# CyberAgentAILab/layout-dm

Hardware: NVIDIA H100
Metric: layouts_per_sec_T100_batch1024_N25 (higher is better)
Workload: dtype fp16

## Files before the change

layoutdm_b200/csrc/common.cuh:

```cuda
#pragma once
#include <cuda.h>
#include <cuda_bf16.h>
#include <cuda_fp16.h>
#include <cuda_runtime.h>
#include <stdint.h>

namespace ldm {

#define LDM_DEVINL __device__ __forceinline__

constexpr float kLogEps = -69.07755278982137f;

LDM_DEVINL uint32_t smem_u32(const void* p) { return static_cast<uint32_t>(__cvta_generic_to_shared(p)); }
LDM_DEVINL void st_shared_u32(uint32_t addr, uint32_t v) { asm volatile("st.shared.u32 [%0], %1;" ::"r"(addr), "r"(v) : "memory"); }

LDM_DEVINL void pdl_wait() { asm volatile("griddepcontrol.wait;" ::: "memory"); }
LDM_DEVINL void pdl_launch_dependents() { asm volatile("griddepcontrol.launch_dependents;" ::: "memory"); }
LDM_DEVINL void pdl_sync() { pdl_wait(); pdl_launch_dependents(); }

LDM_DEVINL void mbar_init(uint64_t* bar, uint32_t count) {
  asm volatile("mbarrier.init.shared::cta.b64 [%0], %1;" ::"r"(smem_u32(bar)), "r"(count) : "memory");
}
LDM_DEVINL void fence_mbar_init() { asm volatile("fence.mbarrier_init.release.cluster;" ::: "memory"); }

// ... 3 lines not shown
LDM_DEVINL void mbar_arrive(uint64_t* bar) {
  asm volatile("mbarrier.arrive.shared::cta.b64 _, [%0];" ::"r"(smem_u32(bar)) : "memory");
}
LDM_DEVINL bool mbar_try_wait(uint64_t* bar, uint32_t parity) {
  uint32_t ok;
  asm volatile(
      "{\n\t.reg .pred p;\n\t"
      "mbarrier.try_wait.parity.shared::cta.b64 p, [%1], %2;\n\t"
      "selp.u32 %0, 1, 0, p;\n\t}\n"
      : "=r"(ok)
      : "r"(smem_u32(bar)), "r"(parity)
      : "memory");
  return ok != 0;
}
LDM_DEVINL void mbar_wait(uint64_t* bar, uint32_t parity) {
  uint32_t spins = 0;
  while (!mbar_try_wait(bar, parity)) {
    if (++spins > (1u << 28)) { asm volatile("trap;"); }
  }
}

LDM_DEVINL void tma_prefetch_desc(const CUtensorMap* m) {
  asm volatile("prefetch.tensormap [%0];" ::"l"(reinterpret_cast<uint64_t>(m)) : "memory");
}
LDM_DEVINL void tma_load_2d(void* smem_dst, const CUtensorMap* map, uint64_t* bar, int32_t c0, int32_t c1) {
  asm volatile(
      "cp.async.bulk.tensor.2d.shared::cluster.global.mbarrier::complete_tx::bytes [%0], [%1, {%3, %4}], [%2];"
      ::"r"(smem_u32(smem_dst)), "l"(reinterpret_cast<uint64_t>(map)), "r"(smem_u32(bar)), "r"(c0), "r"(c1)
      : "memory");
}
LDM_DEVINL void tma_store_2d(const CUtensorMap* map, const void* smem_src, int32_t c0, int32_t c1) {
  asm volatile("cp.async.bulk.tensor.2d.global.shared::cta.bulk_group [%0, {%2, %3}], [%1];"
               ::"l"(reinterpret_cast<uint64_t>(map)), "r"(smem_u32(smem_src)), "r"(c0), "r"(c1)
               : "memory");
}
LDM_DEVINL void bulk_copy_g2s(void* smem_dst, const void* src, uint32_t bytes, uint64_t* bar) {
  asm volatile("cp.async.bulk.shared::cluster.global.mbarrier::complete_tx::bytes [%0], [%1], %2, [%3];"
               ::"r"(smem_u32(smem_dst)), "l"(reinterpret_cast<uint64_t>(src)), "r"(bytes), "r"(smem_u32(bar))
               : "memory");
}
LDM_DEVINL void bulk_copy_s2g(void* dst, const void* smem_src, uint32_t bytes) {
  asm volatile("cp.async.bulk.global.shared::cta.bulk_group [%0], [%1], %2;"
               ::"l"(reinterpret_cast<uint64_t>(dst)), "r"(smem_u32(smem_src)), "r"(bytes)
               : "memory");
}
LDM_DEVINL void bulk_commit_group() { asm volatile("cp.async.bulk.commit_group;" ::: "memory"); }
template <int N>
LDM_DEVINL void bulk_wait_group_read() { asm volatile("cp.async.bulk.wait_group.read %0;" ::"n"(N) : "memory"); }
LDM_DEVINL void bulk_wait_group_all() { asm volatile("cp.async.bulk.wait_group 0;" ::: "memory"); }
LDM_DEVINL void fence_proxy_async_smem() { asm volatile("fence.proxy.async.shared::cta;" ::: "memory"); }

template <int R>
LDM_DEVINL void setmaxnreg_inc() { asm volatile("setmaxnreg.inc.sync.aligned.u32 %0;" ::"n"(R)); }
template <int R>
LDM_DEVINL void setmaxnreg_dec() { asm volatile("setmaxnreg.dec.sync.aligned.u32 %0;" ::"n"(R)); }

LDM_DEVINL uint32_t cluster_ctarank() { uint32_t r; asm volatile("mov.u32 %0, %%cluster_ctarank;" : "=r"(r)); return r; }
LDM_DEVINL uint32_t cluster_id_x() { uint32_t r; asm volatile("mov.u32 %0, %%clusterid.x;" : "=r"(r)); return r; }
LDM_DEVINL uint32_t cluster_count_x() { uint32_t r; asm volatile("mov.u32 %0, %%nclusterid.x;" : "=r"(r)); return r; }
LDM_DEVINL void cluster_sync() {
  asm volatile("barrier.cluster.arrive.release;\n\tbarrier.cluster.wait.acquire;" ::: "memory");
}
LDM_DEVINL uint32_t map_peer(const void* p, uint32_t rank) {
  uint32_t r;
  asm volatile("mapa.shared::cluster.u32 %0, %1, %2;" : "=r"(r) : "r"(smem_u32(p)), "r"(rank));
  return r;
}
LDM_DEVINL void st_async_f32(uint32_t addr, float v, uint32_t bar) {
  asm volatile("st.async.shared::cluster.mbarrier::complete_tx::bytes.f32 [%0], %1, [%2];" ::"r"(addr), "f"(v), "r"(bar) : "memory");
}

LDM_DEVINL void named_bar_sync(int id, int nthreads) { asm volatile("bar.sync %0, %1;" ::"r"(id), "r"(nthreads) : "memory"); }
LDM_DEVINL void named_bar_arrive(int id, int nthreads) { asm volatile("bar.arrive %0, %1;" ::"r"(id), "r"(nthreads) : "memory"); }

LDM_DEVINL void wgmma_fence() { asm volatile("wgmma.fence.sync.aligned;" ::: "memory"); }
LDM_DEVINL void wgmma_commit() { asm volatile("wgmma.commit_group.sync.aligned;" ::: "memory"); }
// ... 232 lines not shown
```

layoutdm_b200/csrc/gemm_tc.cuh:

```cuda
#pragma once
#include "common.cuh"

namespace ldm {

constexpr int kBM = 128;
constexpr int kWgK = 16;
constexpr int kGemmConsumers = 256;
constexpr int kProducerRegs = 40, kConsumerRegs = 232;

constexpr int gemm_kb(bool split) { return split ? 32 : 64; }

enum : int { EPI_QKV = 0, EPI_RELU = 1, EPI_F32 = 2, EPI_LN = 3 };

struct GemmParams {
  int M, N, K;
  int n_tiles;
  const float* bias;
  void* out;
  int ldo;
  float qscale;
  int qcols;
  const float* resid;
  float* y_out;
  const float* ln_scale;
// ... 427 lines not shown
#pragma unroll
      for (int cb = 0; cb < kCols / 64; ++cb) {
        if (n0 + cb * 64 >= p.N) continue;
        if (leader) bulk_wait_group_read<0>();
        wg_bar();
#pragma unroll
        for (int j8 = 8 * cb; j8 < 8 * cb + 8; ++j8) {
          const int c = col0 + 8 * j8;
          const uint32_t blk = stage_u32 + ((((j8 & 7) << 4) ^ sw) | (4 * (lane & 3)));
#pragma unroll
          for (int h = 0; h < 2; ++h) {
            float v[4];
            bias_act<EPI>(acc[h], j8, p.bias, c, scale, v);
            st_shared_u32(blk + (h * 64 + rw) * 128, O::pack(v[0], v[1]));
            st_shared_u32(blk + (h * 64 + rw + 8) * 128, O::pack(v[2], v[3]));
          }
        }
        fence_proxy_async_smem();
        wg_bar();
        if (leader) {
          tma_store_2d(&map_out, stage, n0 + cb * 64, m0);
          bulk_commit_group();
        }
      }
    }
    if (!mine_any) {
      for (int kb = 0; kb < num_kb; ++kb) { mbar_wait(&a_full[kb], ip); mbar_arrive(&a_empty[kb]); }
    }
  }
  if (leader) bulk_wait_group_all();
}

constexpr int kLnThreads = 384, kLnEpiThreads = 96;
template <int STAGES>
struct LnSmem {
  static constexpr int kRows = kBM, kCols = 232, kPairCols = 2 * kCols;
  using R = Ring<32, 1, kRows, kCols, 1, STAGES, false>;
  static constexpr int kLd = kCols;
  static constexpr int kOffBuf = R::kBytes;
  static constexpr int kOffBars = kOffBuf + kRows * kLd * 4;
  static constexpr int kOffStat = kOffBars + 128;
  static constexpr int kBytes = kOffStat + 9 * kRows * 4 + 1024 ;
  static_assert(2 * R::kStages * 8 + 6 * 8 <= 128, "barrier block overflow");
  static_assert(kLd * 4 % 16 == 0 && kLd * 4 % 128 == 32, "bulk copies need 16-byte aligned rows; fragment accesses need rows 32 mod 128 bytes");
  static_assert(kRows * kCols * 4 < (1 << 20), "a tile's residual bytes exceed the mbarrier transaction count");
};

template <int MODE, int STAGES>
__global__ void __launch_bounds__(kLnThreads, 1)
gemm_ln_kernel(const __grid_constant__ OpMaps<MODE> map_a , const __grid_constant__ OpMaps<MODE> map_b ,
               const GemmParams p) {
  static_assert(!kOpSplit<MODE>, "the split mode runs the fragment-epilogue LN GEMM");
  using SM = LnSmem<STAGES>;
  using O = OpT<MODE>;
  constexpr int kRows = SM::kRows, kCols = SM::kCols, kLd = SM::kLd, kAcc = kCols / 2;
  constexpr int kEpi = kGemmConsumers, kProducer = kEpi + kLnEpiThreads;

  extern __shared__ __align__(1024) uint8_t smem_raw[];
  uint8_t* smem = reinterpret_cast<uint8_t*>((reinterpret_cast<uintptr_t>(smem_raw) + 1023) & ~uintptr_t(1023));
  typename SM::R ring(smem, reinterpret_cast<uint64_t*>(smem + SM::kOffBars));
  uint64_t* res_full = ring.empty + SM::R::kStages;
  uint64_t* buf_full = res_full + 1;
  uint64_t* xs_full = buf_full + 1;
  uint64_t* xv_full = xs_full + 2;
  float* buf = reinterpret_cast<float*>(smem + SM::kOffBuf);
  float* s_piv = reinterpret_cast<float*>(smem + SM::kOffStat);
  float* s_own = s_piv + kRows;
  float* s_sum = s_own + kRows;
  float* v_own = s_sum + kRows;
  float* s_rstd = v_own + kRows;
  float* x_sum = s_rstd + kRows;
  float* x_var = x_sum + 2 * kRows;

  const int warp = __shfl_sync(0xffffffffu, threadIdx.x >> 5, 0), lane = threadIdx.x & 31;
  const int N = p.N;
  const int num_kb = SM::R::num_kb(p.K);
  const int n_work = p.M / kRows;
  const uint32_t rank = cluster_ctarank();
  const int col0 = kCols * static_cast<int>(rank);
  const int cl = static_cast<int>(cluster_id_x()), n_cl = static_cast<int>(cluster_count_x());
  const auto tile_m0 = [&](int t) { return (p.rev ? n_work - 1 - t : t) * kRows; };
  const uint32_t peer = rank ^ 1;
  const uint32_t px_sum = map_peer(x_sum, peer), pxs_full = map_peer(xs_full, peer);

  if (threadIdx.x == kProducer) {
    ring.prefetch(map_a, map_b);
    ring.init();
    mbar_init(res_full, 1);
    mbar_init(buf_full, kGemmConsumers);
    for (int b = 0; b < 2; ++b) { mbar_init(&xs_full[b], 1); mbar_init(&xv_full[b], 1); }
    fence_mbar_init();
  }
  cluster_sync();
  pdl_sync();

  if (threadIdx.x >= kProducer) {
    if (threadIdx.x == kProducer) {
      uint32_t phase = 0;
      int s = 0;
      for (int t = cl; t < n_work; t += n_cl) ring.load_tile(s, phase, map_a, map_b, num_kb, tile_m0(t), col0);
    }
  } else if (threadIdx.x >= kEpi) {
    const int et = threadIdx.x - kEpi;
    const bool copier = et < 32;
    constexpr uint32_t kRowBytes = kCols * sizeof(float);
    const float inv_n = 1.0f / static_cast<float>(N);
    constexpr int kVec = kCols / 4;
    constexpr int kTotal = kRows * kVec;
    constexpr int kPerThread = (kTotal + kLnEpiThreads - 1) / kLnEpiThreads;
    const uint32_t px_var = map_peer(x_var, peer), pxv_full = map_peer(xv_full, peer);
    const auto load_resid = [&](int t) {
      if (lane == 0) mbar_arrive_expect_tx(res_full, kRows * kRowBytes);
      __syncwarp();
      const float* src = p.resid + static_cast<size_t>(tile_m0(t)) * N + col0;
      for (int r = lane; r < kRows; r += 32) bulk_copy_g2s(buf + r * kLd, src + static_cast<size_t>(r) * N, kRowBytes, res_full);
    };
    const auto store_rows = [&](float* dst) {
      for (int r = lane; r < kRows; r += 32) bulk_copy_s2g(dst + static_cast<size_t>(r) * N, buf + r * kLd, kRowBytes);
      bulk_commit_group();
    };
    if (copier) load_resid(cl);
    uint32_t bphase = 0;
    int it = 0;
    for (int t = cl; t < n_work; t += n_cl, ++it) {
      const int m0 = tile_m0(t), b = it & 1;
      const uint32_t xph = (it >> 1) & 1;
      if (et == 0) { mbar_arrive_expect_tx(&xs_full[b], kRows * 4); mbar_arrive_expect_tx(&xv_full[b], kRows * 4); }
      mbar_wait(buf_full, bphase);
      if (copier && p.y_out != nullptr) store_rows(p.y_out + static_cast<size_t>(m0) * N + col0);
      const int q = lane & 3;
      mbar_wait(&xs_full[b], xph);
#pragma unroll 1
      for (int g = et >> 5; g < kRows / 8; g += kLnEpiThreads / 32) {
        const int r = 8 * g + (lane >> 2);
        const float piv = s_piv[r], s = s_own[r] + x_sum[b * kRows + r];
        const float* yr = buf + r * kLd + 2 * q;
        float v = 0.0f;
#pragma unroll
        for (int j = 0; j < kCols / 8; ++j) {
          const float2 y = *reinterpret_cast<const float2*>(yr + 8 * j);
          const float d0 = fmaf(-s, inv_n, y.x - piv), d1 = fmaf(-s, inv_n, y.y - piv);
          v = fmaf(d0, d0, fmaf(d1, d1, v));
        }
        v += __shfl_xor_sync(0xffffffffu, v, 1);
        v += __shfl_xor_sync(0xffffffffu, v, 2);
        if (q == 0) { s_sum[r] = s; v_own[r] = v; st_async_f32(px_var + (b * kRows + r) * 4, v, pxv_full + b * 8); }
      }
      mbar_wait(&xv_full[b], xph);
      if (q == 0) {
#pragma unroll 1
        for (int g = et >> 5; g < kRows / 8; g += kLnEpiThreads / 32) {
          const int r = 8 * g + (lane >> 2);
          s_rstd[r] = 1.0f / sqrtf(fmaxf((v_own[r] + x_var[b * kRows + r]) * inv_n, 0.0f) + 1e-5f);
        }
      }
      if (copier) bulk_wait_group_read<0>();
      named_bar_sync(1, kLnEpiThreads);
      const LnAffine a = ln_affine(p.ln_scale, p.ln_shift, p.adaln, p.t_layout, p.n_layouts, m0, N);
      const float *gam = a.gam + col0, *bet = a.bet + col0;
      typename O::T* out16 = static_cast<typename O::T*>(p.out) + col0;
      const bool keep32 = p.out32 != nullptr;
#pragma unroll 6
      for (int k = 0; k < kPerThread; ++k) {
        const int i = k * kLnEpiThreads + et, r = i / kVec, c = (i - r * kVec) * 4;
        if (i >= kTotal) continue;
        float4* bp = reinterpret_cast<float4*>(buf + r * kLd + c);
        const float4 y = *bp;
        const float4 g = __ldg(reinterpret_cast<const float4*>(gam + c)), h = __ldg(reinterpret_cast<const float4*>(bet + c));
        const float piv = s_piv[r], s = s_sum[r], rstd = s_rstd[r];
        const float4 v = make_float4(fmaf(fmaf(-s, inv_n, y.x - piv) * rstd, g.x + a.gadd, h.x), fmaf(fmaf(-s, inv_n, y.y - piv) * rstd, g.y + a.gadd, h.y),
                                     fmaf(fmaf(-s, inv_n, y.z - piv) * rstd, g.z + a.gadd, h.z), fmaf(fmaf(-s, inv_n, y.w - piv) * rstd, g.w + a.gadd, h.w));
        *reinterpret_cast<uint2*>(out16 + static_cast<size_t>(m0 + r) * N + c) = make_uint2(O::pack(v.x, v.y), O::pack(v.z, v.w));
        if (keep32) *bp = v;
      }
      if (keep32) fence_proxy_async_smem();
      named_bar_sync(1, kLnEpiThreads);
      if (copier) {
        if (keep32) store_rows(p.out32 + static_cast<size_t>(m0) * N + col0);
        bulk_wait_group_read<0>();
        if (t + n_cl < n_work) load_resid(t + n_cl);
      }
      bphase ^= 1;
    }
    if (copier) bulk_wait_group_all();
  } else {
    const int wg = warp >> 2;
    float acc[kAcc];
    int s = 0;
    uint32_t phase = 0, bphase = 0;
    const int rw = 64 * wg + (warp & 3) * 16 + (lane >> 2);
    const int cw = 2 * (lane & 3);
    const float* bias = p.bias + col0;
    float* bw = buf + rw * kLd + cw;
    int it = 0;
    for (int t = cl; t < n_work; t += n_cl, ++it) {
      const int m0 = tile_m0(t);
      ring.template mma_tile<MODE>(s, phase, acc, wg, 0, num_kb, p.K);
      float piv0 = 0.0f, piv1 = 0.0f;
      if (cw == 0) {
        const float b0 = __ldg(p.bias);
        piv0 = b0 + p.resid[static_cast<size_t>(m0 + rw) * N];
        piv1 = b0 + p.resid[static_cast<size_t>(m0 + rw + 8) * N];
      }
      piv0 = __shfl_sync(0xffffffffu, piv0, lane & ~3);
      piv1 = __shfl_sync(0xffffffffu, piv1, lane & ~3);
      mbar_wait(res_full, bphase);
      if (cw == 0) { s_piv[rw] = piv0; s_piv[rw + 8] = piv1; }
      float s0 = 0.0f, s1 = 0.0f;
#pragma unroll
      for (int j = 0; j < kAcc / 4; ++j) {
        const float2 b = __ldg(reinterpret_cast<const float2*>(bias + cw + 8 * j));
        float2* y0 = reinterpret_cast<float2*>(bw + 8 * j);
        float2* y1 = reinterpret_cast<float2*>(bw + 8 * kLd + 8 * j);
        const float2 r0 = *y0, r1 = *y1;
        const float2 v0 = make_float2(acc[4 * j] + (b.x + r0.x), acc[4 * j + 1] + (b.y + r0.y));
        const float2 v1 = make_float2(acc[4 * j + 2] + (b.x + r1.x), acc[4 * j + 3] + (b.y + r1.y));
        *y0 = v0;
        *y1 = v1;
        s0 += (v0.x - piv0) + (v0.y - piv0);
        s1 += (v1.x - piv1) + (v1.y - piv1);
      }
      s0 += __shfl_xor_sync(0xffffffffu, s0, 1);
      s1 += __shfl_xor_sync(0xffffffffu, s1, 1);
      s0 += __shfl_xor_sync(0xffffffffu, s0, 2);
      s1 += __shfl_xor_sync(0xffffffffu, s1, 2);
      if (cw == 0) {
        const int b = it & 1;
        s_own[rw] = s0; s_own[rw + 8] = s1;
        st_async_f32(px_sum + (b * kRows + rw) * 4, s0, pxs_full + b * 8);
        st_async_f32(px_sum + (b * kRows + rw + 8) * 4, s1, pxs_full + b * 8);
      }
      fence_proxy_async_smem();
      mbar_arrive(buf_full);
      bphase ^= 1;
    }
  }
  cluster_sync();
}

}
```

layoutdm_b200/csrc/ldm_b200.cu:

```cuda
#include <cuda.h>
#include <cuda_runtime.h>

#include <algorithm>
#include <cmath>
#include <cstdarg>
#include <cstdio>
#include <cstdlib>
#include <cstring>
#include <type_traits>
#include <vector>

#include "../../include/ldm_b200.h"
#include "attention.cuh"
#include "common.cuh"
#include "embed.cuh"
#include "gemm_tc.cuh"
#include "posterior_sample.cuh"
#include "relation.cuh"

using namespace ldm;

namespace {

thread_local char g_err[512] = "";
// ... 31 lines not shown
template <int MODE> constexpr auto kGemmHead = gemm_tc_kernel<kHeadBN, 2, kHeadStages, EPI_F32, MODE>;
template <int MODE> constexpr auto kGemmLn = gemm_tc_kernel<kLnBN, 1, kLnStages, EPI_LN, MODE>;
constexpr int kPlainSmem = GemmSmem<kPlainBN, 2, kPlainStages, true>::kBytes;
constexpr int kHeadSmem = GemmSmem<kHeadBN, 2, kHeadStages>::kBytes;
constexpr int kLnSmem = GemmSmem<kLnBN, 1, kLnStages>::kBytes;
static_assert(GemmSmem<kHeadBN, 2, kHeadStages, true>::kBytes == kHeadSmem && GemmSmem<kLnBN, 1, kLnStages, true>::kBytes == kLnSmem,
              "split-mode ring stages must keep the one-plane sizes");

using EncodeTiledFn = CUresult (*)(CUtensorMap*, CUtensorMapDataType, cuuint32_t, void*, const cuuint64_t*, const cuuint64_t*,
                                   const cuuint32_t*, const cuuint32_t*, CUtensorMapInterleave, CUtensorMapSwizzle,
                                   CUtensorMapL2promotion, CUtensorMapFloatOOBfill);
EncodeTiledFn g_encode = nullptr;

int load_encode() {
  if (g_encode) return LDM_OK;
  void* fn = nullptr;
  cudaDriverEntryPointQueryResult qres;
  CK(cudaGetDriverEntryPoint("cuTensorMapEncodeTiled", &fn, cudaEnableDefault, &qres));
  if (qres != cudaDriverEntryPointSuccess || fn == nullptr) return fail(LDM_ERR_CUDA, "cuTensorMapEncodeTiled not available");
  g_encode = reinterpret_cast<EncodeTiledFn>(fn);
  return LDM_OK;
}

int make_map(CUtensorMap* m, const void* base, uint64_t rows, uint64_t cols, uint32_t box_rows, int kb, bool bf16) {
  const cuuint64_t dims[2] = {cols, rows};
  const cuuint64_t strides[1] = {cols * 2};
  const cuuint32_t box[2] = {static_cast<cuuint32_t>(kb), box_rows};
  const cuuint32_t estr[2] = {1, 1};
  CUresult r = g_encode(m, bf16 ? CU_TENSOR_MAP_DATA_TYPE_BFLOAT16 : CU_TENSOR_MAP_DATA_TYPE_FLOAT16, 2, const_cast<void*>(base), dims,
                        strides, box, estr, CU_TENSOR_MAP_INTERLEAVE_NONE, kb == 32 ? CU_TENSOR_MAP_SWIZZLE_64B : CU_TENSOR_MAP_SWIZZLE_128B,
                        CU_TENSOR_MAP_L2_PROMOTION_L2_256B, CU_TENSOR_MAP_FLOAT_OOB_FILL_NONE);
  if (r != CUDA_SUCCESS) return fail(LDM_ERR_CUDA, "cuTensorMapEncodeTiled failed (%d) rows=%llu cols=%llu box_rows=%u", (int)r,
                                     (unsigned long long)rows, (unsigned long long)cols, box_rows);
  return LDM_OK;
}

__global__ void logits_scatter_kernel(const float* __restrict__ src, float* __restrict__ dst, int n_layouts, int S, int C) {
  const size_t n = static_cast<size_t>(n_layouts) * S * C;
  for (size_t i = blockIdx.x * static_cast<size_t>(blockDim.x) + threadIdx.x; i < n; i += static_cast<size_t>(gridDim.x) * blockDim.x) {
    const int c = static_cast<int>(i % C); const size_t tok = i / C; const int s = static_cast<int>(tok % S); const size_t b = tok / S;
    dst[(b * 128 + s) * kLogitLd + c] = src[i];
  }
}
__global__ void logits_gather_kernel(const float* __restrict__ src, float* __restrict__ dst, int n_layouts, int S, int C) {
  const size_t n = static_cast<size_t>(n_layouts) * S * C;
  for (size_t i = blockIdx.x * static_cast<size_t>(blockDim.x) + threadIdx.x; i < n; i += static_cast<size_t>(gridDim.x) * blockDim.x) {
    const int c = static_cast<int>(i % C); const size_t tok = i / C; const int s = static_cast<int>(tok % S); const size_t b = tok / S;
    dst[i] = src[(b * 128 + s) * kLogitLd + c];
  }
}
__global__ void fill_ids_kernel(long long* dst, long long v, size_t n) {
  for (size_t i = blockIdx.x * static_cast<size_t>(blockDim.x) + threadIdx.x; i < n; i += static_cast<size_t>(gridDim.x) * blockDim.x) dst[i] = v;
}

}

struct LdmHandle {
  LdmModelDesc desc;
  int C = 0, S = 0, L = 0, T = 0, G = 0;
  int mode = OP_F16;
  bool bf16 = false;
  bool split = false;
  int64_t launches = 0;
  int pdl = 1;
  int debug_stop_after = 0;
  bool prof = false;
  struct ProfRec { int cat; cudaEvent_t a, b; };
  std::vector<ProfRec> prof_recs;
  float *cat_emb = nullptr, *pos = nullptr, *adaln = nullptr, *sched = nullptr, *lae = nullptr;
  void *wqkv[kMaxLayers] = {}, *wo[kMaxLayers] = {}, *w1[kMaxLayers] = {}, *w2[kMaxLayers] = {}, *whead = nullptr;
  float *bqkv[kMaxLayers] = {}, *bo[kMaxLayers] = {}, *b1[kMaxLayers] = {}, *b2[kMaxLayers] = {}, *ln2w[kMaxLayers] = {}, *ln2b[kMaxLayers] = {};
  float *hlnw = nullptr, *hlnb = nullptr;
  CUtensorMap m_wqkv[kMaxLayers], m_wo[kMaxLayers], m_w1[kMaxLayers], m_w2[kMaxLayers], m_whead;
  void *wqkv_lo[kMaxLayers] = {}, *wo_lo[kMaxLayers] = {}, *w1_lo[kMaxLayers] = {}, *w2_lo[kMaxLayers] = {}, *whead_lo = nullptr;
  CUtensorMap m_wqkv_lo[kMaxLayers], m_wo_lo[kMaxLayers], m_w1_lo[kMaxLayers], m_w2_lo[kMaxLayers], m_whead_lo;
  int *qmap = nullptr, *amap = nullptr, *hmap = nullptr;
  int cap = 0;
  void *x16 = nullptr, *qkv16 = nullptr, *att16 = nullptr, *z16 = nullptr, *hid16 = nullptr;
  float *x32 = nullptr, *y32 = nullptr, *logits = nullptr;
  float* rel_lp = nullptr;
  long long* ids[2] = {nullptr, nullptr};
  long long* ids_final = nullptr;
  long long *c_seq = nullptr, *c_seq_orig = nullptr; unsigned char* c_mask = nullptr; float* c_tbl = nullptr;
  CUtensorMap m_x16, m_z16, m_qkv16;
  CUtensorMap m_att16, m_hid16;
  CUtensorMap m_qkv16_st, m_hid16_st;
  void *x16_lo = nullptr, *qkv16_lo = nullptr, *att16_lo = nullptr, *z16_lo = nullptr, *hid16_lo = nullptr;
  CUtensorMap m_x16_lo, m_z16_lo, m_qkv16_lo, m_att16_lo, m_hid16_lo;
  std::vector<void*> owned;
  int use_graph = 1;
  int sweep = 1;
  int num_sms = 0;
  int max_threads_sm = 0;
  int gemm_ctas = 0;
  int ln_clusters = 0;
  int gemm_split = 0;
  int fuse_embed = 1;
  cudaStream_t cap_stream = nullptr;
  cudaGraphExec_t graph_exec = nullptr;
  uint64_t graph_key = 0;
  unsigned long long* call_block = nullptr;
  uint64_t ws_generation = 0;
  int64_t graph_launches = 0;
  std::vector<void*> staging;
};

namespace {

template <typename T>
int dev_alloc(LdmHandle* h, T** p, size_t n) {
  CK(cudaMalloc(reinterpret_cast<void**>(p), n * sizeof(T)));
  h->owned.push_back(*p);
  return LDM_OK;
}
template <typename T>
int dev_upload(LdmHandle* h, T** p, const T* src, size_t n) {
  int rc = dev_alloc(h, p, n);
  if (rc) return rc;
  CK(cudaMemcpy(*p, src, n * sizeof(T), cudaMemcpyHostToDevice));
// ... 208 lines not shown
  }
  CK(cudaMalloc(&h->x16, M * d * 2));
  CK(cudaMalloc(&h->qkv16, M * kQkvN * 2));
  CK(cudaMalloc(&h->att16, M * kAttN * 2));
  CK(cudaMalloc(&h->z16, M * d * 2));
  CK(cudaMalloc(&h->hid16, M * ff * 2));
  CK(cudaMalloc(reinterpret_cast<void**>(&h->x32), M * d * 4));
  CK(cudaMalloc(reinterpret_cast<void**>(&h->y32), M * d * 4));
  CK(cudaMalloc(reinterpret_cast<void**>(&h->logits), M * kLogitLd * 4));
  const size_t nid = static_cast<size_t>(n_layouts) * h->S;
  CK(cudaMalloc(reinterpret_cast<void**>(&h->ids[0]), nid * 8));
  CK(cudaMalloc(reinterpret_cast<void**>(&h->ids[1]), nid * 8));
  CK(cudaMalloc(reinterpret_cast<void**>(&h->ids_final), nid * 8));
  CK(cudaMalloc(reinterpret_cast<void**>(&h->c_seq), nid * 8));
  CK(cudaMalloc(reinterpret_cast<void**>(&h->c_seq_orig), nid * 8));
  CK(cudaMalloc(reinterpret_cast<void**>(&h->c_mask), nid));
  CK(cudaMemset(h->x16, 0, M * d * 2)); CK(cudaMemset(h->qkv16, 0, M * kQkvN * 2)); CK(cudaMemset(h->att16, 0, M * kAttN * 2));
  CK(cudaMemset(h->z16, 0, M * d * 2)); CK(cudaMemset(h->hid16, 0, M * ff * 2)); CK(cudaMemset(h->x32, 0, M * d * 4));
  CK(cudaMemset(h->y32, 0, M * d * 4));
  CK(cudaMemset(h->logits, 0, M * kLogitLd * 4));
  h->cap = n_layouts;
  h->ws_generation++;
  int rc;
  static_assert(gemm_kb(false) == RbSmem::kKB, "one A geometry for QKV / FF1 / head");
  const int kb = gemm_kb(h->split);
  if ((rc = make_op_maps(h, &h->m_x16, &h->m_x16_lo, h->x16, h->x16_lo, M, d, kBM, kb))) return rc;
  if ((rc = make_op_maps(h, &h->m_z16, &h->m_z16_lo, h->z16, h->z16_lo, M, d, kBM, kb))) return rc;
  const int ln_rows = h->split ? kLnSplitRows : LnFf2::kRows;
  if ((rc = make_op_maps(h, &h->m_att16, &h->m_att16_lo, h->att16, h->att16_lo, M, kAttN, ln_rows, kLnKB))) return rc;
  if ((rc = make_op_maps(h, &h->m_hid16, &h->m_hid16_lo, h->hid16, h->hid16_lo, M, ff, ln_rows, kLnKB))) return rc;
  if ((rc = make_op_maps(h, &h->m_qkv16, &h->m_qkv16_lo, h->qkv16, h->qkv16_lo, M, kQkvN, kBM, kHeadPad))) return rc;
  if (!h->split && (rc = make_map(&h->m_qkv16_st, h->qkv16, M, kQkvN, kBM, 64, h->bf16))) return rc;
  if (!h->split && (rc = make_map(&h->m_hid16_st, h->hid16, M, ff, kBM, 64, h->bf16))) return rc;
  return LDM_OK;
}

template <int MODE>
int launch_denoiser(LdmHandle* h, int n, const long long* ids_in, int t_model, cudaStream_t st, const int* t_layout = nullptr, bool skip_embed = false) {
  const auto maps = [](const CUtensorMap& hi, const CUtensorMap& lo) { return op_maps<MODE>(hi, lo); };
  const int d = h->desc.d_model, ff = h->desc.d_ff, L = h->L, T = h->T;
  const int M = n * kBM;
  const auto grid = [&](int tiles, bool persistent) {
    if (!persistent) return dim3(tiles);
    return dim3(std::min({tiles, h->num_sms, h->gemm_ctas > 0 ? h->gemm_ctas : tiles}));
  };
  const auto plain_gemm = [&](auto epi, const OpMaps<MODE>& a, const OpMaps<MODE>& w, const CUtensorMap& out, GemmParams p) {
    constexpr int EPI = decltype(epi)::value;
    if constexpr (kOpSplit<MODE>) {
      p.n_tiles = (p.N + kPlainBN - 1) / kPlainBN;
      return launch_step(h, kGemmPlainSplit<EPI, MODE>, grid(p.n_tiles * n, false), kGemmThreads, kPlainSmem, st, a, w, p);
    } else {
      p.n_tiles = (p.N + kRbCols - 1) / kRbCols;
      const int g = h->gemm_split > 0 ? h->gemm_split : n >= h->num_sms ? 1 : (h->num_sms + n - 1) / n;
      p.n_ranges = std::min(g, p.n_tiles);
      return launch_step(h, gemm_rowblock_kernel<EPI, MODE>, grid(n * p.n_ranges, true), kRbThreads, RbSmem::kBytes, st, a, w, out, p);
    }
  };
  const auto ln_gemm = [&](const OpMaps<MODE>& a, const OpMaps<MODE>& w, const GemmParams& p) {
    if constexpr (kOpSplit<MODE>) {
      return launch_step(h, kGemmLn<MODE>, grid(M / kLnSplitRows, false), kGemmThreads, kLnSmem, st, a, w, p);
    } else {
      const int pairs = std::min({n, h->ln_clusters, h->gemm_ctas > 0 ? std::max(1, h->gemm_ctas / 2) : n});
      if (p.K == kAttN) return launch_cluster(h, 2, gemm_ln_kernel<MODE, kLnOutStages>, dim3(2 * pairs), kLnThreads, LnOut::kBytes, st, a, w, p);
      return launch_cluster(h, 2, gemm_ln_kernel<MODE, kLnFf2Stages>, dim3(2 * pairs), kLnThreads, LnFf2::kBytes, st, a, w, p);
    }
  };
  int done = 0;
  int dir = 0;
  auto next_rev = [&]() { dir ^= 1; return h->sweep ? dir : 0; };
#define LDM_STAGE_DONE() do { if (h->debug_stop_after && ++done >= h->debug_stop_after) { CK(cudaGetLastError()); return LDM_OK; } } while (0)
  if (!skip_embed) {
    const int warps = n * 128, blocks = (warps * 32 + 255) / 256;
    ProfScope ps(h, CAT_EMBED, st);
    CK(launch_step(h, embed_adaln_kernel<MODE>, dim3(blocks), 256, 0, st, ids_in, (const float*)h->cat_emb, (const float*)h->pos,
                   (const float*)h->adaln, t_model, t_layout, h->x32, h->x16, n, n, h->S, d, h->x16_lo));
  }
  if (!skip_embed) LDM_STAGE_DONE();
  for (int l = 0; l < L; ++l) {
    {
      GemmParams p{M, kQkvN, d, 0, h->bqkv[l], h->qkv16, kQkvN, 1.0f / sqrtf(static_cast<float>(d / h->desc.n_heads)), 8 * kHeadPad};
      p.rev = next_rev(); p.out_lo = h->qkv16_lo;
      ProfScope ps(h, CAT_QKV, st);
      CK(plain_gemm(std::integral_constant<int, EPI_QKV>{}, maps(h->m_x16, h->m_x16_lo), maps(h->m_wqkv[l], h->m_wqkv_lo[l]), h->m_qkv16_st, p));
    }
    LDM_STAGE_DONE();
    {
      ProfScope ps(h, CAT_ATTN, st);
      CK(launch_step(h, attention_kernel<MODE>, dim3(n * h->desc.n_heads), kAttThreads, kOpSplit<MODE> ? kAttSmemBytesSplit : kAttSmemBytes, st,
                     maps(h->m_qkv16, h->m_qkv16_lo), h->att16, h->S, h->desc.n_heads, n, next_rev(), h->att16_lo));
    }
    LDM_STAGE_DONE();
    {
      GemmParams p{M, d, kAttN, 1, h->bo[l], h->z16, d, 1.0f, 0, h->x32, h->y32, h->ln2w[l], h->ln2b[l], 0, nullptr};
      p.rev = next_rev(); p.out_lo = h->z16_lo;
      ProfScope ps(h, CAT_OUTPROJ, st);
      CK(ln_gemm(maps(h->m_att16, h->m_att16_lo), maps(h->m_wo[l], h->m_wo_lo[l]), p));
    }
    LDM_STAGE_DONE();
    {
      GemmParams p{M, ff, d, 0, h->b1[l], h->hid16, ff, 1.0f, 0};
      p.rev = next_rev(); p.out_lo = h->hid16_lo;
      ProfScope ps(h, CAT_FF1, st);
      CK(plain_gemm(std::integral_constant<int, EPI_RELU>{}, maps(h->m_z16, h->m_z16_lo), maps(h->m_w1[l], h->m_w1_lo[l]), h->m_hid16_st, p));
    }
    LDM_STAGE_DONE();
    {
      GemmParams p{M, d, ff, 1, h->b2[l], nullptr, d, 1.0f, 0, h->y32, nullptr, nullptr, nullptr, 0, nullptr};
      if (l + 1 < L) {
        const float* tab = h->adaln + (static_cast<size_t>(l + 1) * T + t_model) * 2 * d;
        p.ln_scale = tab; p.ln_shift = tab + d; p.adaln = 1; p.out32 = h->x32; p.out = h->x16; p.out_lo = h->x16_lo;
        if (t_layout) { p.ln_scale = h->adaln + static_cast<size_t>(l + 1) * T * 2 * d; p.t_layout = t_layout; p.n_layouts = n; }
      } else {
        p.ln_scale = h->hlnw; p.ln_shift = h->hlnb; p.adaln = 0; p.out32 = nullptr; p.out = h->z16; p.out_lo = h->z16_lo;
      }
      p.rev = next_rev();
      ProfScope ps(h, CAT_FF2, st);
      CK(ln_gemm(maps(h->m_hid16, h->m_hid16_lo), maps(h->m_w2[l], h->m_w2_lo[l]), p));
    }
    LDM_STAGE_DONE();
  }
  {
    GemmParams p{M, kLogitLd, d, 1, nullptr, h->logits, kLogitLd, 1.0f, 0};
    p.rev = next_rev();
    ProfScope ps(h, CAT_HEAD, st);
    CK(launch_step(h, kGemmHead<MODE>, grid(n, false), kGemmThreads, kHeadSmem, st, maps(h->m_z16, h->m_z16_lo), maps(h->m_whead, h->m_whead_lo), p));
  }
#undef LDM_STAGE_DONE
  CK(cudaGetLastError());
  return LDM_OK;
}

int run_denoiser(LdmHandle* h, int n, const long long* ids_in, int t_model, cudaStream_t st, const int* t_layout = nullptr, bool skip_embed = false) {
  switch (h->mode) {
    case OP_BF16X3: return launch_denoiser<OP_BF16X3>(h, n, ids_in, t_model, st, t_layout, skip_embed);
    case OP_BF16: return launch_denoiser<OP_BF16>(h, n, ids_in, t_model, st, t_layout, skip_embed);
    default: return launch_denoiser<OP_F16>(h, n, ids_in, t_model, st, t_layout, skip_embed);
  }
}

int validate_common(LdmHandle* h, int B, const LdmSampling* s) {
  if (!h) return fail(LDM_ERR_INVALID, "null handle");
  if (B <= 0) return fail(LDM_ERR_INVALID, "batch size must be positive (got %d)", B);
  if (!s) return fail(LDM_ERR_INVALID, "null sampling config");
  if (s->mode < 0 || s->mode > LDM_SAMPLING_GUMBEL) return fail(LDM_ERR_INVALID, "unknown sampling mode %d (sampling.py:118 raises NotImplementedError)", s->mode);
  if (s->mode != LDM_SAMPLING_DETERMINISTIC && !(s->temperature > 0.0f)) return fail(LDM_ERR_INVALID, "temperature must be > 0");
  if (s->mode == LDM_SAMPLING_TOP_P && !(s->top_p > 0.0f && s->top_p <= 1.0f)) return fail(LDM_ERR_INVALID, "top_p must be in (0, 1] (sampling.py:96)");
  if (s->mode == LDM_SAMPLING_TOP_K && !(s->top_k >= 1 && s->top_k <= h->C)) return fail(LDM_ERR_INVALID, "top_k out of range");
  return LDM_OK;
}

// ... 606 lines not shown
  v.x0_recon = reinterpret_cast<long long*>(x0_recon_out); v.xtm1_recon = reinterpret_cast<long long*>(xtm1_recon_out);
  const int blocks = (B * h->S * 32 + 255) / 256, rblocks = (B * 32 + 255) / 256;
  { ProfScope ps(h, CAT_EPILOGUE, st); CK(launch_step(h, vb_terms_kernel, blocks, 256, 0, st, v)); }
  { ProfScope ps(h, CAT_MISC, st); CK(launch_step(h, row_mean_kernel, rblocks, 256, 0, st, (const float*)v.kl_tok, kl_out, B, h->S)); }
  { ProfScope ps(h, CAT_MISC, st); CK(launch_step(h, row_mean_kernel, rblocks, 256, 0, st, (const float*)v.nll_tok, nll_out, B, h->S)); }
  if (kl_aux_out) { ProfScope ps(h, CAT_MISC, st); CK(launch_step(h, row_mean_kernel, rblocks, 256, 0, st, (const float*)v.aux_tok, kl_aux_out, B, h->S)); }
  CK(cudaGetLastError());
  return LDM_OK;
}

int64_t ldm_launch_count(const LdmHandle* h) { return h ? h->launches : 0; }

int ldm_profile_begin(LdmHandle* h) {
  if (!h) return fail(LDM_ERR_INVALID, "null handle");
  h->prof = true;
  return LDM_OK;
}

int ldm_profile_end(LdmHandle* h, float* ms_per_category, int64_t* launches_per_category, int32_t n_categories) {
  if (!h) return fail(LDM_ERR_INVALID, "null handle");
  h->prof = false;
  CK(cudaDeviceSynchronize());
  for (int i = 0; i < n_categories; ++i) { if (ms_per_category) ms_per_category[i] = 0.0f; if (launches_per_category) launches_per_category[i] = 0; }
  for (auto& r : h->prof_recs) {
    float ms = 0.0f;
    cudaEventElapsedTime(&ms, r.a, r.b);
    if (r.cat < n_categories) { if (ms_per_category) ms_per_category[r.cat] += ms; if (launches_per_category) launches_per_category[r.cat]++; }
    cudaEventDestroy(r.a); cudaEventDestroy(r.b);
  }
  h->prof_recs.clear();
  return LDM_OK;
}

int ldm_debug_set_stop_after(LdmHandle* h, int32_t n_launches) {
  if (!h) return fail(LDM_ERR_INVALID, "null handle");
  h->debug_stop_after = n_launches;
  return LDM_OK;
}

int64_t ldm_debug_read(const LdmHandle* h, const char* name, void* dst, int64_t capacity_bytes, int32_t n_layouts) {
  if (!h || !name || n_layouts > h->cap) return -1;
  const size_t M = static_cast<size_t>(n_layouts) * kBM;
  const int d = h->desc.d_model, ff = h->desc.d_ff;
  const void* src = nullptr; size_t bytes = 0;
  if (!strcmp(name, "x32")) { src = h->x32; bytes = M * d * 4; }
  else if (!strcmp(name, "y32")) { src = h->y32; bytes = M * d * 4; }
  else if (!strcmp(name, "x16")) { src = h->x16; bytes = M * d * 2; }
  else if (!strcmp(name, "z16")) { src = h->z16; bytes = M * d * 2; }
  else if (!strcmp(name, "att16")) { src = h->att16; bytes = M * kAttN * 2; }
  else if (!strcmp(name, "qkv16")) { src = h->qkv16; bytes = M * kQkvN * 2; }
  else if (!strcmp(name, "hid16")) { src = h->hid16; bytes = M * ff * 2; }
  else if (!strcmp(name, "logits")) { src = h->logits; bytes = M * kLogitLd * 4; }
  else if (!strcmp(name, "x16_lo")) { src = h->x16_lo; bytes = M * d * 2; }
  else if (!strcmp(name, "z16_lo")) { src = h->z16_lo; bytes = M * d * 2; }
  else if (!strcmp(name, "att16_lo")) { src = h->att16_lo; bytes = M * kAttN * 2; }
  else if (!strcmp(name, "qkv16_lo")) { src = h->qkv16_lo; bytes = M * kQkvN * 2; }
  else if (!strcmp(name, "hid16_lo")) { src = h->hid16_lo; bytes = M * ff * 2; }
  else return -1;
  if (!h->split && strstr(name, "_lo") != nullptr) return -1;
  if (dst && capacity_bytes >= static_cast<int64_t>(bytes)) {
    if (cudaDeviceSynchronize() != cudaSuccess) return -2;
    if (cudaMemcpy(dst, src, bytes, cudaMemcpyDeviceToHost) != cudaSuccess) return -2;
  }
  return static_cast<int64_t>(bytes);
}
int32_t ldm_num_classes(const LdmHandle* h) { return h ? h->C : 0; }
// ... 17 lines not shown
```

Before: 1092.

## Split LN GEMM epilogue into row halves and use TMA for residual traffic

The LayerNorm GEMM epilogue now processes each 128-row tile as two 64-row halves, each with its own barriers, so the epilogue warps can start on one half while the other warpgroup is still producing its half. Residual loads and fp32 stores switch from per-row bulk copies issued by a whole warp to 2D TMA tensor-map loads and stores issued by one thread, using new fp32 tensor maps. A compile-time timing probe is also added but stays off by default. The finer split adds more barrier waits and more bookkeeping in exchange for overlap.

```diff
diff --git a/layoutdm_b200/csrc/common.cuh b/layoutdm_b200/csrc/common.cuh
--- a/layoutdm_b200/csrc/common.cuh
+++ b/layoutdm_b200/csrc/common.cuh
@@ -59,16 +59,6 @@
 LDM_DEVINL void tma_store_2d(const CUtensorMap* map, const void* smem_src, int32_t c0, int32_t c1) {
   asm volatile("cp.async.bulk.tensor.2d.global.shared::cta.bulk_group [%0, {%2, %3}], [%1];"
                ::"l"(reinterpret_cast<uint64_t>(map)), "r"(smem_u32(smem_src)), "r"(c0), "r"(c1)
-               : "memory");
-}
-LDM_DEVINL void bulk_copy_g2s(void* smem_dst, const void* src, uint32_t bytes, uint64_t* bar) {
-  asm volatile("cp.async.bulk.shared::cluster.global.mbarrier::complete_tx::bytes [%0], [%1], %2, [%3];"
-               ::"r"(smem_u32(smem_dst)), "l"(reinterpret_cast<uint64_t>(src)), "r"(bytes), "r"(smem_u32(bar))
-               : "memory");
-}
-LDM_DEVINL void bulk_copy_s2g(void* dst, const void* smem_src, uint32_t bytes) {
-  asm volatile("cp.async.bulk.global.shared::cta.bulk_group [%0], [%1], %2;"
-               ::"l"(reinterpret_cast<uint64_t>(dst)), "r"(smem_u32(smem_src)), "r"(bytes)
                : "memory");
 }
 LDM_DEVINL void bulk_commit_group() { asm volatile("cp.async.bulk.commit_group;" ::: "memory"); }
diff --git a/layoutdm_b200/csrc/gemm_tc.cuh b/layoutdm_b200/csrc/gemm_tc.cuh
--- a/layoutdm_b200/csrc/gemm_tc.cuh
+++ b/layoutdm_b200/csrc/gemm_tc.cuh
@@ -483,44 +483,61 @@
 }
 
 constexpr int kLnThreads = 384, kLnEpiThreads = 96;
+
+enum : int { LNP_MAIN = 0, LNP_RES, LNP_Y, LNP_BUF, LNP_XS, LNP_XV, LNP_NORM, LNP_WAIT, LNP_NEXT, LNP_N };
+constexpr int kLnProbePairs = 8, kLnProbeTiles = 32;
+#ifdef LDM_LN_PROBE
+__device__ unsigned long long g_ln_probe[2][kLnProbePairs][kLnProbeTiles][2][LNP_N];
+#endif
+LDM_DEVINL void ln_probe(int K, uint32_t rank, int cl, int it, int half, int stamp) {
+#ifdef LDM_LN_PROBE
+  if (rank == 0 && cl < kLnProbePairs && it < kLnProbeTiles) {
+    unsigned long long t;
+    asm volatile("mov.u64 %0, %%globaltimer;" : "=l"(t));
+    g_ln_probe[K == 512 ? 0 : 1][cl][it][half][stamp] = t;
+  }
+#endif
+}
+
 template <int STAGES>
 struct LnSmem {
-  static constexpr int kRows = kBM, kCols = 232, kPairCols = 2 * kCols;
+  static constexpr int kRows = kBM, kHalf = kRows / 2, kCols = 232, kPairCols = 2 * kCols;
   using R = Ring<32, 1, kRows, kCols, 1, STAGES, false>;
   static constexpr int kLd = kCols;
   static constexpr int kOffBuf = R::kBytes;
   static constexpr int kOffBars = kOffBuf + kRows * kLd * 4;
-  static constexpr int kOffStat = kOffBars + 128;
-  static constexpr int kBytes = kOffStat + 9 * kRows * 4 + 1024 ;
-  static_assert(2 * R::kStages * 8 + 6 * 8 <= 128, "barrier block overflow");
-  static_assert(kLd * 4 % 16 == 0 && kLd * 4 % 128 == 32, "bulk copies need 16-byte aligned rows; fragment accesses need rows 32 mod 128 bytes");
-  static_assert(kRows * kCols * 4 < (1 << 20), "a tile's residual bytes exceed the mbarrier transaction count");
+  static constexpr int kOffStat = kOffBars + 256;
+  static constexpr int kBytes = kOffStat + 8 * kRows * 4 + 1024 ;
+  static_assert(2 * R::kStages * 8 + 12 * 8 <= 256, "barrier block overflow");
+  static_assert(kLd * 4 % 16 == 0 && kHalf * kLd * 4 % 128 == 0 && kLd * 4 % 128 == 32,
+                "TMA boxes need 16-byte multiple rows and 128-byte aligned halves; fragment accesses need rows 32 mod 128 bytes");
+  static_assert(kHalf * kCols * 4 < (1 << 20), "a row half's residual bytes exceed the mbarrier transaction count");
 };
 
 template <int MODE, int STAGES>
 __global__ void __launch_bounds__(kLnThreads, 1)
 gemm_ln_kernel(const __grid_constant__ OpMaps<MODE> map_a , const __grid_constant__ OpMaps<MODE> map_b ,
-               const GemmParams p) {
+               const __grid_constant__ CUtensorMap map_res ,
+               const __grid_constant__ CUtensorMap map_st , const GemmParams p) {
   static_assert(!kOpSplit<MODE>, "the split mode runs the fragment-epilogue LN GEMM");
   using SM = LnSmem<STAGES>;
   using O = OpT<MODE>;
-  constexpr int kRows = SM::kRows, kCols = SM::kCols, kLd = SM::kLd, kAcc = kCols / 2;
+  constexpr int kRows = SM::kRows, kHalf = SM::kHalf, kCols = SM::kCols, kLd = SM::kLd, kAcc = kCols / 2;
   constexpr int kEpi = kGemmConsumers, kProducer = kEpi + kLnEpiThreads;
 
   extern __shared__ __align__(1024) uint8_t smem_raw[];
   uint8_t* smem = reinterpret_cast<uint8_t*>((reinterpret_cast<uintptr_t>(smem_raw) + 1023) & ~uintptr_t(1023));
   typename SM::R ring(smem, reinterpret_cast<uint64_t*>(smem + SM::kOffBars));
   uint64_t* res_full = ring.empty + SM::R::kStages;
-  uint64_t* buf_full = res_full + 1;
-  uint64_t* xs_full = buf_full + 1;
-  uint64_t* xv_full = xs_full + 2;
+  uint64_t* buf_full = res_full + 2;
+  uint64_t* xs_full = buf_full + 2;
+  uint64_t* xv_full = xs_full + 4;
   float* buf = reinterpret_cast<float*>(smem + SM::kOffBuf);
   float* s_piv = reinterpret_cast<float*>(smem + SM::kOffStat);
   float* s_own = s_piv + kRows;
   float* s_sum = s_own + kRows;
-  float* v_own = s_sum + kRows;
-  float* s_rstd = v_own + kRows;
-  float* x_sum = s_rstd + kRows;
+  float* s_var = s_sum + kRows;
+  float* x_sum = s_var + kRows;
   float* x_var = x_sum + 2 * kRows;
 
   const int warp = __shfl_sync(0xffffffffu, threadIdx.x >> 5, 0), lane = threadIdx.x & 31;
@@ -536,10 +553,11 @@
 
   if (threadIdx.x == kProducer) {
     ring.prefetch(map_a, map_b);
+    tma_prefetch_desc(&map_res);
+    tma_prefetch_desc(&map_st);
     ring.init();
-    mbar_init(res_full, 1);
-    mbar_init(buf_full, kGemmConsumers);
-    for (int b = 0; b < 2; ++b) { mbar_init(&xs_full[b], 1); mbar_init(&xv_full[b], 1); }
+    for (int w = 0; w < 2; ++w) { mbar_init(&res_full[w], 1); mbar_init(&buf_full[w], kGemmConsumers / 2); }
+    for (int x = 0; x < 4; ++x) { mbar_init(&xs_full[x], 1); mbar_init(&xv_full[x], 1); }
     fence_mbar_init();
   }
   cluster_sync();
@@ -553,83 +571,90 @@
     }
   } else if (threadIdx.x >= kEpi) {
     const int et = threadIdx.x - kEpi;
-    const bool copier = et < 32;
-    constexpr uint32_t kRowBytes = kCols * sizeof(float);
+    const bool copier = et == 0;
+    constexpr uint32_t kHalfBytes = kHalf * kCols * sizeof(float);
     const float inv_n = 1.0f / static_cast<float>(N);
     constexpr int kVec = kCols / 4;
-    constexpr int kTotal = kRows * kVec;
+    constexpr int kTotal = kHalf * kVec;
     constexpr int kPerThread = (kTotal + kLnEpiThreads - 1) / kLnEpiThreads;
     const uint32_t px_var = map_peer(x_var, peer), pxv_full = map_peer(xv_full, peer);
-    const auto load_resid = [&](int t) {
-      if (lane == 0) mbar_arrive_expect_tx(res_full, kRows * kRowBytes);
-      __syncwarp();
-      const float* src = p.resid + static_cast<size_t>(tile_m0(t)) * N + col0;
-      for (int r = lane; r < kRows; r += 32) bulk_copy_g2s(buf + r * kLd, src + static_cast<size_t>(r) * N, kRowBytes, res_full);
+    const auto load_resid = [&](int t, int w) {
+      mbar_arrive_expect_tx(&res_full[w], kHalfBytes);
+      tma_load_2d(buf + kHalf * w * kLd, &map_res, &res_full[w], col0, tile_m0(t) + kHalf * w);
     };
-    const auto store_rows = [&](float* dst) {
-      for (int r = lane; r < kRows; r += 32) bulk_copy_s2g(dst + static_cast<size_t>(r) * N, buf + r * kLd, kRowBytes);
+    const auto store_rows = [&](int m0, int w) {
+      tma_store_2d(&map_st, buf + kHalf * w * kLd, col0, m0 + kHalf * w);
       bulk_commit_group();
     };
-    if (copier) load_resid(cl);
+    if (copier) { load_resid(cl, 0); load_resid(cl, 1); }
     uint32_t bphase = 0;
     int it = 0;
     for (int t = cl; t < n_work; t += n_cl, ++it) {
       const int m0 = tile_m0(t), b = it & 1;
       const uint32_t xph = (it >> 1) & 1;
-      if (et == 0) { mbar_arrive_expect_tx(&xs_full[b], kRows * 4); mbar_arrive_expect_tx(&xv_full[b], kRows * 4); }
-      mbar_wait(buf_full, bphase);
-      if (copier && p.y_out != nullptr) store_rows(p.y_out + static_cast<size_t>(m0) * N + col0);
-      const int q = lane & 3;
-      mbar_wait(&xs_full[b], xph);
-#pragma unroll 1
-      for (int g = et >> 5; g < kRows / 8; g += kLnEpiThreads / 32) {
-        const int r = 8 * g + (lane >> 2);
-        const float piv = s_piv[r], s = s_own[r] + x_sum[b * kRows + r];
-        const float* yr = buf + r * kLd + 2 * q;
-        float v = 0.0f;
-#pragma unroll
-        for (int j = 0; j < kCols / 8; ++j) {
-          const float2 y = *reinterpret_cast<const float2*>(yr + 8 * j);
-          const float d0 = fmaf(-s, inv_n, y.x - piv), d1 = fmaf(-s, inv_n, y.y - piv);
-          v = fmaf(d0, d0, fmaf(d1, d1, v));
-        }
-        v += __shfl_xor_sync(0xffffffffu, v, 1);
-        v += __shfl_xor_sync(0xffffffffu, v, 2);
-        if (q == 0) { s_sum[r] = s; v_own[r] = v; st_async_f32(px_var + (b * kRows + r) * 4, v, pxv_full + b * 8); }
-      }
-      mbar_wait(&xv_full[b], xph);
-      if (q == 0) {
-#pragma unroll 1
-        for (int g = et >> 5; g < kRows / 8; g += kLnEpiThreads / 32) {
-          const int r = 8 * g + (lane >> 2);
-          s_rstd[r] = 1.0f / sqrtf(fmaxf((v_own[r] + x_var[b * kRows + r]) * inv_n, 0.0f) + 1e-5f);
-        }
-      }
-      if (copier) bulk_wait_group_read<0>();
-      named_bar_sync(1, kLnEpiThreads);
       const LnAffine a = ln_affine(p.ln_scale, p.ln_shift, p.adaln, p.t_layout, p.n_layouts, m0, N);
       const float *gam = a.gam + col0, *bet = a.bet + col0;
       typename O::T* out16 = static_cast<typename O::T*>(p.out) + col0;
       const bool keep32 = p.out32 != nullptr;
+#pragma unroll 1
+      for (int w = 0; w < 2; ++w) {
+        const int h0 = kHalf * w, x = 2 * b + w;
+        if (et == 0) { mbar_arrive_expect_tx(&xs_full[x], kHalf * 4); mbar_arrive_expect_tx(&xv_full[x], kHalf * 4); }
+        mbar_wait(&buf_full[w], bphase);
+        if (et == 0) ln_probe(p.K, rank, cl, it, w, LNP_BUF);
+        if (copier && p.y_out != nullptr) store_rows(m0, w);
+        const int q = lane & 3;
+        mbar_wait(&xs_full[x], xph);
+        if (et == 0) ln_probe(p.K, rank, cl, it, w, LNP_XS);
+#pragma unroll 1
+        for (int g = et >> 5; g < kHalf / 8; g += kLnEpiThreads / 32) {
+          const int r = h0 + 8 * g + (lane >> 2);
+          const float piv = s_piv[r], s = s_own[r] + x_sum[b * kRows + r];
+          const float* yr = buf + r * kLd + 2 * q;
+          float v = 0.0f;
+#pragma unroll
+          for (int j = 0; j < kCols / 8; ++j) {
+            const float2 y = *reinterpret_cast<const float2*>(yr + 8 * j);
+            const float d0 = fmaf(-s, inv_n, y.x - piv), d1 = fmaf(-s, inv_n, y.y - piv);
+            v = fmaf(d0, d0, fmaf(d1, d1, v));
+          }
+          v += __shfl_xor_sync(0xffffffffu, v, 1);
+          v += __shfl_xor_sync(0xffffffffu, v, 2);
+          if (q == 0) { s_sum[r] = s; s_var[r] = v; st_async_f32(px_var + (b * kRows + r) * 4, v, pxv_full + x * 8); }
+        }
+        mbar_wait(&xv_full[x], xph);
+        if (et == 0) ln_probe(p.K, rank, cl, it, w, LNP_XV);
+        if (q == 0) {
+#pragma unroll 1
+          for (int g = et >> 5; g < kHalf / 8; g += kLnEpiThreads / 32) {
+            const int r = h0 + 8 * g + (lane >> 2);
+            s_var[r] = 1.0f / sqrtf(fmaxf((s_var[r] + x_var[b * kRows + r]) * inv_n, 0.0f) + 1e-5f);
+          }
+        }
+        named_bar_sync(1, kLnEpiThreads);
 #pragma unroll 6
-      for (int k = 0; k < kPerThread; ++k) {
-        const int i = k * kLnEpiThreads + et, r = i / kVec, c = (i - r * kVec) * 4;
-        if (i >= kTotal) continue;
-        float4* bp = reinterpret_cast<float4*>(buf + r * kLd + c);
-        const float4 y = *bp;
-        const float4 g = __ldg(reinterpret_cast<const float4*>(gam + c)), h = __ldg(reinterpret_cast<const float4*>(bet + c));
-        const float piv = s_piv[r], s = s_sum[r], rstd = s_rstd[r];
-        const float4 v = make_float4(fmaf(fmaf(-s, inv_n, y.x - piv) * rstd, g.x + a.gadd, h.x), fmaf(fmaf(-s, inv_n, y.y - piv) * rstd, g.y + a.gadd, h.y),
-                                     fmaf(fmaf(-s, inv_n, y.z - piv) * rstd, g.z + a.gadd, h.z), fmaf(fmaf(-s, inv_n, y.w - piv) * rstd, g.w + a.gadd, h.w));
-        *reinterpret_cast<uint2*>(out16 + static_cast<size_t>(m0 + r) * N + c) = make_uint2(O::pack(v.x, v.y), O::pack(v.z, v.w));
-        if (keep32) *bp = v;
-      }
-      if (keep32) fence_proxy_async_smem();
-      named_bar_sync(1, kLnEpiThreads);
-      if (copier) {
-        if (keep32) store_rows(p.out32 + static_cast<size_t>(m0) * N + col0);
-        bulk_wait_group_read<0>();
-        if (t + n_cl < n_work) load_resid(t + n_cl);
+        for (int k = 0; k < kPerThread; ++k) {
+          const int i = k * kLnEpiThreads + et, r = h0 + i / kVec, c = (i - (r - h0) * kVec) * 4;
+          if (i >= kTotal) continue;
+          float4* bp = reinterpret_cast<float4*>(buf + r * kLd + c);
+          const float4 y = *bp;
+          const float4 g = __ldg(reinterpret_cast<const float4*>(gam + c)), h = __ldg(reinterpret_cast<const float4*>(bet + c));
+          const float piv = s_piv[r], s = s_sum[r], rstd = s_var[r];
+          const float4 v = make_float4(fmaf(fmaf(-s, inv_n, y.x - piv) * rstd, g.x + a.gadd, h.x), fmaf(fmaf(-s, inv_n, y.y - piv) * rstd, g.y + a.gadd, h.y),
+                                       fmaf(fmaf(-s, inv_n, y.z - piv) * rstd, g.z + a.gadd, h.z), fmaf(fmaf(-s, inv_n, y.w - piv) * rstd, g.w + a.gadd, h.w));
+          *reinterpret_cast<uint2*>(out16 + static_cast<size_t>(m0 + r) * N + c) = make_uint2(O::pack(v.x, v.y), O::pack(v.z, v.w));
+          if (keep32) *bp = v;
+        }
+        if (keep32) fence_proxy_async_smem();
+        named_bar_sync(1, kLnEpiThreads);
+        if (et == 0) ln_probe(p.K, rank, cl, it, w, LNP_NORM);
+        if (copier) {
+          if (keep32) store_rows(m0, w);
+          bulk_wait_group_read<0>();
+          if (et == 0) ln_probe(p.K, rank, cl, it, w, LNP_WAIT);
+          if (t + n_cl < n_work) load_resid(t + n_cl, w);
+          if (et == 0) ln_probe(p.K, rank, cl, it, w, LNP_NEXT);
+        }
       }
       bphase ^= 1;
     }
@@ -639,7 +664,7 @@
     float acc[kAcc];
     int s = 0;
     uint32_t phase = 0, bphase = 0;
-    const int rw = 64 * wg + (warp & 3) * 16 + (lane >> 2);
+    const int rw = kHalf * wg + (warp & 3) * 16 + (lane >> 2);
     const int cw = 2 * (lane & 3);
     const float* bias = p.bias + col0;
     float* bw = buf + rw * kLd + cw;
@@ -647,6 +672,7 @@
     for (int t = cl; t < n_work; t += n_cl, ++it) {
       const int m0 = tile_m0(t);
       ring.template mma_tile<MODE>(s, phase, acc, wg, 0, num_kb, p.K);
+      if (threadIdx.x % 128 == 0) ln_probe(p.K, rank, cl, it, wg, LNP_MAIN);
       float piv0 = 0.0f, piv1 = 0.0f;
       if (cw == 0) {
         const float b0 = __ldg(p.bias);
@@ -655,7 +681,8 @@
       }
       piv0 = __shfl_sync(0xffffffffu, piv0, lane & ~3);
       piv1 = __shfl_sync(0xffffffffu, piv1, lane & ~3);
-      mbar_wait(res_full, bphase);
+      mbar_wait(&res_full[wg], bphase);
+      if (threadIdx.x % 128 == 0) ln_probe(p.K, rank, cl, it, wg, LNP_RES);
       if (cw == 0) { s_piv[rw] = piv0; s_piv[rw + 8] = piv1; }
       float s0 = 0.0f, s1 = 0.0f;
 #pragma unroll
@@ -676,13 +703,14 @@
       s0 += __shfl_xor_sync(0xffffffffu, s0, 2);
       s1 += __shfl_xor_sync(0xffffffffu, s1, 2);
       if (cw == 0) {
-        const int b = it & 1;
+        const int b = it & 1, x = 2 * b + wg;
         s_own[rw] = s0; s_own[rw + 8] = s1;
-        st_async_f32(px_sum + (b * kRows + rw) * 4, s0, pxs_full + b * 8);
-        st_async_f32(px_sum + (b * kRows + rw + 8) * 4, s1, pxs_full + b * 8);
+        st_async_f32(px_sum + (b * kRows + rw) * 4, s0, pxs_full + x * 8);
+        st_async_f32(px_sum + (b * kRows + rw + 8) * 4, s1, pxs_full + x * 8);
       }
       fence_proxy_async_smem();
-      mbar_arrive(buf_full);
+      mbar_arrive(&buf_full[wg]);
+      if (threadIdx.x % 128 == 0) ln_probe(p.K, rank, cl, it, wg, LNP_Y);
       bphase ^= 1;
     }
   }
diff --git a/layoutdm_b200/csrc/ldm_b200.cu b/layoutdm_b200/csrc/ldm_b200.cu
--- a/layoutdm_b200/csrc/ldm_b200.cu
+++ b/layoutdm_b200/csrc/ldm_b200.cu
@@ -87,6 +87,18 @@
                         CU_TENSOR_MAP_L2_PROMOTION_L2_256B, CU_TENSOR_MAP_FLOAT_OOB_FILL_NONE);
   if (r != CUDA_SUCCESS) return fail(LDM_ERR_CUDA, "cuTensorMapEncodeTiled failed (%d) rows=%llu cols=%llu box_rows=%u", (int)r,
                                      (unsigned long long)rows, (unsigned long long)cols, box_rows);
+  return LDM_OK;
+}
+
+int make_map_f32(CUtensorMap* m, const void* base, uint64_t rows, uint64_t cols, uint32_t box_rows, uint32_t box_cols) {
+  const cuuint64_t dims[2] = {cols, rows};
+  const cuuint64_t strides[1] = {cols * 4};
+  const cuuint32_t box[2] = {box_cols, box_rows};
+  const cuuint32_t estr[2] = {1, 1};
+  CUresult r = g_encode(m, CU_TENSOR_MAP_DATA_TYPE_FLOAT32, 2, const_cast<void*>(base), dims, strides, box, estr, CU_TENSOR_MAP_INTERLEAVE_NONE,
+                        CU_TENSOR_MAP_SWIZZLE_NONE, CU_TENSOR_MAP_L2_PROMOTION_L2_256B, CU_TENSOR_MAP_FLOAT_OOB_FILL_NONE);
+  if (r != CUDA_SUCCESS) return fail(LDM_ERR_CUDA, "cuTensorMapEncodeTiled failed (%d) fp32 rows=%llu cols=%llu box %u x %u", (int)r,
+                                     (unsigned long long)rows, (unsigned long long)cols, box_rows, box_cols);
   return LDM_OK;
 }
 
@@ -140,6 +152,7 @@
   CUtensorMap m_x16, m_z16, m_qkv16;
   CUtensorMap m_att16, m_hid16;
   CUtensorMap m_qkv16_st, m_hid16_st;
+  CUtensorMap m_x32, m_y32;
   void *x16_lo = nullptr, *qkv16_lo = nullptr, *att16_lo = nullptr, *z16_lo = nullptr, *hid16_lo = nullptr;
   CUtensorMap m_x16_lo, m_z16_lo, m_qkv16_lo, m_att16_lo, m_hid16_lo;
   std::vector<void*> owned;
@@ -414,6 +427,8 @@
   if ((rc = make_op_maps(h, &h->m_qkv16, &h->m_qkv16_lo, h->qkv16, h->qkv16_lo, M, kQkvN, kBM, kHeadPad))) return rc;
   if (!h->split && (rc = make_map(&h->m_qkv16_st, h->qkv16, M, kQkvN, kBM, 64, h->bf16))) return rc;
   if (!h->split && (rc = make_map(&h->m_hid16_st, h->hid16, M, ff, kBM, 64, h->bf16))) return rc;
+  if (!h->split && (rc = make_map_f32(&h->m_x32, h->x32, M, d, LnFf2::kHalf, kLnBN))) return rc;
+  if (!h->split && (rc = make_map_f32(&h->m_y32, h->y32, M, d, LnFf2::kHalf, kLnBN))) return rc;
   return LDM_OK;
 }
 
@@ -438,13 +453,13 @@
       return launch_step(h, gemm_rowblock_kernel<EPI, MODE>, grid(n * p.n_ranges, true), kRbThreads, RbSmem::kBytes, st, a, w, out, p);
     }
   };
-  const auto ln_gemm = [&](const OpMaps<MODE>& a, const OpMaps<MODE>& w, const GemmParams& p) {
+  const auto ln_gemm = [&](const OpMaps<MODE>& a, const OpMaps<MODE>& w, const CUtensorMap& res, const CUtensorMap& st32, const GemmParams& p) {
     if constexpr (kOpSplit<MODE>) {
       return launch_step(h, kGemmLn<MODE>, grid(M / kLnSplitRows, false), kGemmThreads, kLnSmem, st, a, w, p);
     } else {
       const int pairs = std::min({n, h->ln_clusters, h->gemm_ctas > 0 ? std::max(1, h->gemm_ctas / 2) : n});
-      if (p.K == kAttN) return launch_cluster(h, 2, gemm_ln_kernel<MODE, kLnOutStages>, dim3(2 * pairs), kLnThreads, LnOut::kBytes, st, a, w, p);
-      return launch_cluster(h, 2, gemm_ln_kernel<MODE, kLnFf2Stages>, dim3(2 * pairs), kLnThreads, LnFf2::kBytes, st, a, w, p);
+      if (p.K == kAttN) return launch_cluster(h, 2, gemm_ln_kernel<MODE, kLnOutStages>, dim3(2 * pairs), kLnThreads, LnOut::kBytes, st, a, w, res, st32, p);
+      return launch_cluster(h, 2, gemm_ln_kernel<MODE, kLnFf2Stages>, dim3(2 * pairs), kLnThreads, LnFf2::kBytes, st, a, w, res, st32, p);
     }
   };
   int done = 0;
@@ -476,7 +491,7 @@
       GemmParams p{M, d, kAttN, 1, h->bo[l], h->z16, d, 1.0f, 0, h->x32, h->y32, h->ln2w[l], h->ln2b[l], 0, nullptr};
       p.rev = next_rev(); p.out_lo = h->z16_lo;
       ProfScope ps(h, CAT_OUTPROJ, st);
-      CK(ln_gemm(maps(h->m_att16, h->m_att16_lo), maps(h->m_wo[l], h->m_wo_lo[l]), p));
+      CK(ln_gemm(maps(h->m_att16, h->m_att16_lo), maps(h->m_wo[l], h->m_wo_lo[l]), h->m_x32, h->m_y32, p));
     }
     LDM_STAGE_DONE();
     {
@@ -497,7 +512,7 @@
       }
       p.rev = next_rev();
       ProfScope ps(h, CAT_FF2, st);
-      CK(ln_gemm(maps(h->m_hid16, h->m_hid16_lo), maps(h->m_w2[l], h->m_w2_lo[l]), p));
+      CK(ln_gemm(maps(h->m_hid16, h->m_hid16_lo), maps(h->m_w2[l], h->m_w2_lo[l]), h->m_y32, h->m_x32, p));
     }
     LDM_STAGE_DONE();
   }
@@ -1170,6 +1185,16 @@
   return LDM_OK;
 }
 
+#ifdef LDM_LN_PROBE
+int64_t ldm_probe_ln_read(void* dst, int64_t capacity_bytes) {
+  const int64_t bytes = sizeof(g_ln_probe);
+  if (!dst || capacity_bytes < bytes) return -1;
+  if (cudaDeviceSynchronize() != cudaSuccess || cudaMemcpyFromSymbol(dst, g_ln_probe, bytes) != cudaSuccess) return -1;
+  static const unsigned char zeros[sizeof(g_ln_probe)] = {};
+  return cudaMemcpyToSymbol(g_ln_probe, zeros, bytes) == cudaSuccess ? bytes : -1;
+}
+#endif
+
 int ldm_debug_set_stop_after(LdmHandle* h, int32_t n_launches) {
   if (!h) return fail(LDM_ERR_INVALID, "null handle");
   h->debug_stop_after = n_launches;
```

Result: faster. 1160 (median of 6 runs) (+6.2%).
